# likojack/bnv_fusion

Hardware: AMD Instinct MI355X
Metric: depth frames/sec fused+decoded, 640x480 @ 256^3 grid (higher is better)
Workload: dtype f32 operands split into f16 hi+lo, 3 products on v_mfma_f32_16x16x32_f16, f32 accumulate

## Files before the change

### bnv_fusion_amd/csrc/encode.hip

```cpp
#include <stddef.h>

#include <atomic>
#include <utility>
#include <vector>

#include "frontend.hpp"

namespace bnv {

int g_num_cus = 0;
int g_last_hip_error = 0;
std::atomic<int> g_reserve_cus{0};
std::atomic<int> g_finalize_blocks{0};
std::atomic<int> g_tcnn_shared_table{1};
std::atomic<int> g_tcnn_block_encoder{1};
std::atomic<int> g_mlp_mode{1};

bool g_prof_on = false;
static std::vector<std::pair<hipEvent_t, hipEvent_t>> g_prof_events[PROF_KINDS];
static size_t g_prof_used[PROF_KINDS] = {0, 0, 0, 0};

void prof_mark(int kind, bool begin, hipStream_t stream) {
  auto& ring = g_prof_events[kind];
  if (begin) {
// ... 754 lines not shown
    lo[q] = (uint32_t)__builtin_fmaf(hf, -kFixedScale, r);
  }
#define BNV_SCAN_STEP(ctrl)                                                      \
  "v_add_co_u32_dpp %0, vcc, %0, %0 " ctrl "\n"                                  \
  "v_addc_co_u32_dpp %1, vcc, %1, %1, vcc " ctrl "\n"                            \
  "v_add_co_u32_dpp %2, vcc, %2, %2 " ctrl "\n"                                  \
  "v_addc_co_u32_dpp %3, vcc, %3, %3, vcc " ctrl "\n"                            \
  "v_add_co_u32_dpp %4, vcc, %4, %4 " ctrl "\n"                                  \
  "v_addc_co_u32_dpp %5, vcc, %5, %5, vcc " ctrl "\n"                            \
  "v_add_co_u32_dpp %6, vcc, %6, %6 " ctrl "\n"                                  \
  "v_addc_co_u32_dpp %7, vcc, %7, %7, vcc " ctrl "\n"
  asm volatile("s_nop 1\n"
               BNV_SCAN_STEP("row_shr:1 row_mask:0xf bank_mask:0xf bound_ctrl:1")
               BNV_SCAN_STEP("row_shr:2 row_mask:0xf bank_mask:0xf bound_ctrl:1")
               BNV_SCAN_STEP("row_shr:4 row_mask:0xf bank_mask:0xf bound_ctrl:1")
               BNV_SCAN_STEP("row_shr:8 row_mask:0xf bank_mask:0xf bound_ctrl:1")
               BNV_SCAN_STEP("row_bcast:15 row_mask:0xa bank_mask:0xf")
               : "+v"(lo[0]), "+v"(hi[0]), "+v"(lo[1]), "+v"(hi[1]), "+v"(lo[2]), "+v"(hi[2]), "+v"(lo[3]), "+v"(hi[3])
               :
               : "vcc");
#undef BNV_SCAN_STEP
  const int prev = __builtin_amdgcn_update_dpp(0, slot, 0x138 , 0xf, 0xf, false);
  const unsigned long long heads64 = __ballot(j == 0 || prev != slot);
  const uint32_t heads = h ? (uint32_t)(heads64 >> 32) : (uint32_t)heads64;
  const int s = 31 - __clz((int)(heads & (0xffffffffu >> (31 - j))));
  is_end = j == 31 || ((heads >> (j + 1)) & 1u);
  len = j - s + 1;
  const int src = (h * 32 + (s > 0 ? s - 1 : 0)) * 4;
#pragma unroll
  for (int q = 0; q < 4; ++q) {
    const uint32_t plo = (uint32_t)__builtin_amdgcn_ds_bpermute(src, (int)lo[q]);
    const uint32_t phi = (uint32_t)__builtin_amdgcn_ds_bpermute(src, (int)hi[q]);
    v[q] = ((unsigned long long)hi[q] << 32) | lo[q];
    if (s > 0) v[q] -= ((unsigned long long)phi << 32) | plo;
  }
}

__device__ __forceinline__ void scatter_tile(const f32x16& o, int slot, int j, int h, int32_t* __restrict__ counts,
                                             long long* __restrict__ acc) {
  unsigned long long v[4];
  bool is_end;
  int len;
  tile_run_sums(o, slot, j, h, v, is_end, len);
#ifdef BNV_PROBE_NO_SCATTER
  if ((blockIdx.x & 63) != 0) return;
#endif
  if (slot >= 0 && is_end) {
    unsigned long long* dst = (unsigned long long*)acc + ((uint32_t)slot * 8u + 4u * (uint32_t)h);
#pragma unroll
    for (int q = 0; q < 4; ++q) atomicAdd(dst + q, v[q]);
    if (h == 0) atomicAdd(&counts[slot], len);
  }
}

__global__ __launch_bounds__(512, 2) void k_pointnet_scatter(
    const float* __restrict__ pts, int n_points, bnv_grid_t g, const float* __restrict__ wpack,
    const uint32_t* __restrict__ bitmap, const uint32_t* __restrict__ word_prefix,
    int32_t* __restrict__ counts, long long* __restrict__ acc, const int32_t* __restrict__ pair_list,
    const int32_t* __restrict__ n_pairs) {
  extern __shared__ __attribute__((aligned(16))) float lds[];
  stage_to_lds<512>(wpack, lds, PN_TOTAL * 4);
  __syncthreads();

  const int lane = threadIdx.x & 63;
  const int wave = __builtin_amdgcn_readfirstlane(threadIdx.x >> 6);
  const int j = lane & 31, h = lane >> 5;
  const PairTiles T = pair_tiles(n_points, pair_list, n_pairs);
  const int n_tiles = T.n_tiles;
  const int nyz = g.n_xyz[1] * g.n_xyz[2];

  for (int t = blockIdx.x * 8 + wave; t < n_tiles; t += gridDim.x * 8) {
    int i = 0, k = 0;
    const bool have = tile_pair(T, t, j, &i, &k);
    float in0 = 0.f, in1 = 0.f, in2 = 0.f;
    int slot = -1;
    bool valid = false;
    if (have) {
      const float* p = pts + (size_t)i * 6;
      const float x = p[0], y = p[1], z = p[2];
      valid = in_bounds(x, y, z, g);
      if (valid) {
        const float xn = voxel_coord(x, g.bound_min[0], g.voxel_size);
        const float yn = voxel_coord(y, g.bound_min[1], g.voxel_size);
        const float zn = voxel_coord(z, g.bound_min[2], g.voxel_size);
        const int gx = (k & 1) ? (int)ceilf(xn) : (int)floorf(xn);
        const int gy = (k & 2) ? (int)ceilf(yn) : (int)floorf(yn);
        const int gz = (k & 4) ? (int)ceilf(zn) : (int)floorf(zn);
        if (voxel_owner(gx, gy, gz, g) == g.shard_rank) {
          const uint32_t id = (uint32_t)(gx * nyz + gy * g.n_xyz[2] + gz);
          const uint32_t word = bitmap[id >> 5];
          slot = (int)(word_prefix[id >> 5] + __popc(word & ((1u << (id & 31)) - 1u)));
        }
        const float rx = relative_coord(xn, gx, g.voxel_size);
        const float ry = relative_coord(yn, gy, g.voxel_size);
        const float rz = relative_coord(zn, gz, g.voxel_size);
        in0 = h ? ry : rx;
        in1 = h ? p[3] : rz;
        in2 = h ? p[5] : p[4];
      }
    }
    if (__ballot(slot >= 0) == 0ULL) continue;

    f32x16 ha[4], hb[4];
#pragma unroll
    for (int mb = 0; mb < 4; ++mb) ha[mb] = bias_init(lds + PN_B1, mb, h);
    {
      const float bin[3] = {in0, in1, in2};
#pragma unroll
      for (int s = 0; s < 3; ++s) {
#pragma unroll
        for (int mb = 0; mb < 4; ++mb)
          ha[mb] = __builtin_amdgcn_mfma_f32_32x32x2f32(lds[PN_W1 + (s * 4 + mb) * 64 + lane], bin[s],
                                                        ha[mb], 0, 0, 0);
      }
    }
#pragma unroll
    for (int mb = 0; mb < 4; ++mb) ha[mb] = relu16(ha[mb]);
    layer128(lds + PN_W2, lds + PN_B2, ha, hb, lane, h);
#pragma unroll
    for (int mb = 0; mb < 4; ++mb) hb[mb] = relu16(hb[mb]);
    layer128(lds + PN_W3, lds + PN_B3, hb, ha, lane, h);
#pragma unroll
    for (int mb = 0; mb < 4; ++mb) ha[mb] = relu16(ha[mb]);
    f32x16 o;
#pragma unroll
    for (int r = 0; r < 16; ++r) o[r] = 0.f;
    {
      const f32x4 b4 = *(const f32x4*)&lds[PN_B4 + 4 * h];
#pragma unroll
      for (int r = 0; r < 4; ++r) o[r] = b4[r];
    }
#pragma unroll
    for (int nb = 0; nb < 4; ++nb) {
#pragma unroll
      for (int rq = 0; rq < 4; ++rq) {
        f32x4 a = {0.f, 0.f, 0.f, 0.f};
        if (j < 8) a = *(const f32x4*)&lds[PN_W4 + ((((nb * 4 + rq) * 2 + h) * 8) + j) * 4];
#pragma unroll
        for (int i = 0; i < 4; ++i)
          o = __builtin_amdgcn_mfma_f32_32x32x2f32(a[i], ha[nb][4 * rq + i], o, 0, 0, 0);
      }
    }
    scatter_tile(o, slot, j, h, counts, acc);
  }
}


typedef _Float16 half8 __attribute__((ext_vector_type(8)));

typedef __attribute__((address_space(3))) const half8 lds_half8_t;
typedef __attribute__((address_space(3))) const f32x4 lds_f32x4_t;
constexpr int kLdsWin = 61440;

#ifdef BNV_PHASE_PROF
__device__ unsigned long long g_enc_phase[8 * 16];
#define BNV_EPH(i)                                                                          \
  do {                                                                                      \
    if ((threadIdx.x & 63) == 0) {                                                          \
      unsigned long long* _p = (unsigned long long*)((char*)lds + PX_LDS_BYTES) + (threadIdx.x >> 6) * 16; \
      const unsigned long long _t = clock64();                                              \
      _p[i] += _t - _p[15];                                                                 \
      _p[15] = _t;                                                                          \
    }                                                                                       \
  } while (0)
constexpr int kEncProfLds = 8 * 16 * 8;
#else
#define BNV_EPH(i)
constexpr int kEncProfLds = 0;
#endif

struct EncLdsX {
  uint32_t w[3];
  uint32_t b;
};
__device__ __forceinline__ half8 ldsx_wfrag(const EncLdsX& L, int byte_off) {
  const int b = byte_off / kLdsWin;
  return *(lds_half8_t*)((b == 0 ? L.w[0] : (b == 1 ? L.w[1] : L.w[2])) + (uint32_t)(byte_off - b * kLdsWin));
}
__device__ __forceinline__ f32x4 ldsx_bias(const EncLdsX& L, int layer, int rb) {
  return *(lds_f32x4_t*)(L.b + (uint32_t)((layer * 128 + rb * 16) * 4));
}

template <int NPROD>
__device__ __forceinline__ void layer128_x(const EncLdsX& L, int w_off, int layer, const half8 (&inh)[4][2],
                                           const half8 (&inl)[4][2], f32x4 (&out)[8][2]) {
#pragma unroll
  for (int rb = 0; rb < 8; ++rb) out[rb][0] = out[rb][1] = ldsx_bias(L, layer, rb);
  half8 ah[2], al[2];
#define BNV_LOAD_WX(q)                                                        \
  {                                                                           \
    const int wb = (w_off + (q) * 2 * 64 * 8) * 2;                            \
    ah[(q) & 1] = ldsx_wfrag(L, wb);                                          \
    if (NPROD == 3) al[(q) & 1] = ldsx_wfrag(L, wb + 1024);                   \
  }
  BNV_LOAD_WX(0);
#pragma unroll
  for (int q = 0; q < 32; ++q) {
    if (q + 1 < 32) BNV_LOAD_WX(q + 1);
    __builtin_amdgcn_sched_barrier(0);
    const int s = q >> 3, rb = q & 7;
    if constexpr (NPROD == 3) {
      out[rb][0] = __builtin_amdgcn_mfma_f32_16x16x32_f16(al[q & 1], inh[s][0], out[rb][0], 0, 0, 0);
      out[rb][1] = __builtin_amdgcn_mfma_f32_16x16x32_f16(al[q & 1], inh[s][1], out[rb][1], 0, 0, 0);
      out[rb][0] = __builtin_amdgcn_mfma_f32_16x16x32_f16(ah[q & 1], inl[s][0], out[rb][0], 0, 0, 0);
      out[rb][1] = __builtin_amdgcn_mfma_f32_16x16x32_f16(ah[q & 1], inl[s][1], out[rb][1], 0, 0, 0);
    }
    out[rb][0] = __builtin_amdgcn_mfma_f32_16x16x32_f16(ah[q & 1], inh[s][0], out[rb][0], 0, 0, 0);
    out[rb][1] = __builtin_amdgcn_mfma_f32_16x16x32_f16(ah[q & 1], inh[s][1], out[rb][1], 0, 0, 0);
    __builtin_amdgcn_sched_barrier(0);
  }
#undef BNV_LOAD_WX
}

template <int NPROD>
__device__ __forceinline__ void split_x(const f32x4 (&acc)[8][2], half8 (&oh)[4][2], half8 (&ol)[4][2]) {
#pragma unroll
  for (int s = 0; s < 4; ++s)
#pragma unroll
    for (int cb = 0; cb < 2; ++cb) {
      float x[8];
#pragma unroll
      for (int e = 0; e < 8; ++e) x[e] = relu_bits(acc[2 * s + (e >> 2)][cb][e & 3]);
      if (NPROD == 3) {
        split8_f16(x, oh[s][cb], ol[s][cb]);
      } else {
#pragma unroll
        for (int e = 0; e < 8; ++e) oh[s][cb][e] = (_Float16)x[e];
      }
    }
}

__device__ __forceinline__ void scatter_tile_x(const f32x4& o, int slot, int n, int g, int32_t* __restrict__ counts,
                                               long long* __restrict__ acc) {
  uint32_t lo[4], hi[4];
#pragma unroll
  for (int q = 0; q < 4; ++q) {
    const float r = __builtin_rintf(o[q] * kFixedScale);
    const float hf = __builtin_floorf(r * (1.0f / kFixedScale));
    hi[q] = (uint32_t)(int)hf;
    lo[q] = (uint32_t)__builtin_fmaf(hf, -kFixedScale, r);
  }
#define BNV_SCAN_STEP(ctrl)                                                      \
  "v_add_co_u32_dpp %0, vcc, %0, %0 " ctrl "\n"                                  \
  "v_addc_co_u32_dpp %1, vcc, %1, %1, vcc " ctrl "\n"                            \
  "v_add_co_u32_dpp %2, vcc, %2, %2 " ctrl "\n"                                  \
  "v_addc_co_u32_dpp %3, vcc, %3, %3, vcc " ctrl "\n"                            \
  "v_add_co_u32_dpp %4, vcc, %4, %4 " ctrl "\n"                                  \
  "v_addc_co_u32_dpp %5, vcc, %5, %5, vcc " ctrl "\n"                            \
  "v_add_co_u32_dpp %6, vcc, %6, %6 " ctrl "\n"                                  \
  "v_addc_co_u32_dpp %7, vcc, %7, %7, vcc " ctrl "\n"
  asm volatile("s_nop 1\n"
               BNV_SCAN_STEP("row_shr:1 row_mask:0xf bank_mask:0xf bound_ctrl:1")
               BNV_SCAN_STEP("row_shr:2 row_mask:0xf bank_mask:0xf bound_ctrl:1")
               BNV_SCAN_STEP("row_shr:4 row_mask:0xf bank_mask:0xf bound_ctrl:1")
               BNV_SCAN_STEP("row_shr:8 row_mask:0xf bank_mask:0xf bound_ctrl:1")
               : "+v"(lo[0]), "+v"(hi[0]), "+v"(lo[1]), "+v"(hi[1]), "+v"(lo[2]), "+v"(hi[2]), "+v"(lo[3]), "+v"(hi[3])
               :
               : "vcc");
#undef BNV_SCAN_STEP
  {
    const int tsrc = ((g & 1) * 16 + 15) * 4;
#pragma unroll
    for (int q = 0; q < 4; ++q) {
      const uint32_t tl = (uint32_t)__builtin_amdgcn_ds_bpermute(tsrc, (int)lo[q]);
      const uint32_t th = (uint32_t)__builtin_amdgcn_ds_bpermute(tsrc, (int)hi[q]);
      if (g >= 2) {
        const unsigned long long v = (((unsigned long long)hi[q] << 32) | lo[q]) + (((unsigned long long)th << 32) | tl);
        lo[q] = (uint32_t)v;
        hi[q] = (uint32_t)(v >> 32);
      }
    }
  }
  const int p = (g >> 1) * 16 + n;
  const int slot15 = __builtin_amdgcn_readlane(slot, 15);
  const int prev_row = __builtin_amdgcn_update_dpp(0, slot, 0x111 , 0xf, 0xf, false);
  const int prev = n == 0 ? slot15 : prev_row;
  const unsigned long long heads64 = __ballot(p == 0 || prev != slot);
  const uint32_t heads = ((uint32_t)heads64 & 0xffffu) | (((uint32_t)(heads64 >> 32) & 0xffffu) << 16);
  const int s = 31 - __clz((int)(heads & (0xffffffffu >> (31 - p))));
  const bool is_end = p == 31 || ((heads >> (p + 1)) & 1u);
  const int sp = s > 0 ? s - 1 : 0;
  const int src = (((sp >> 4) * 2 + (g & 1)) * 16 + (sp & 15)) * 4;
  uint32_t plo[4], phi[4];
#pragma unroll
  for (int q = 0; q < 4; ++q) {
    plo[q] = (uint32_t)__builtin_amdgcn_ds_bpermute(src, (int)lo[q]);
    phi[q] = (uint32_t)__builtin_amdgcn_ds_bpermute(src, (int)hi[q]);
  }
#ifdef BNV_PROBE_NO_SCATTER
  if ((blockIdx.x & 63) != 0) return;
#endif
  if (slot >= 0 && is_end) {
    unsigned long long* dst = (unsigned long long*)acc + ((uint32_t)slot * 8u + 4u * (uint32_t)(g & 1));
#pragma unroll
    for (int q = 0; q < 4; ++q) {
      unsigned long long v = ((unsigned long long)hi[q] << 32) | lo[q];
      if (s > 0) v -= ((unsigned long long)phi[q] << 32) | plo[q];
      atomicAdd(dst + q, v);
    }
    if ((g & 1) == 0) atomicAdd(&counts[slot], p - s + 1);
  }
}

template <int NPROD>
__global__ __launch_bounds__(512, 2) __attribute__((amdgpu_num_vgpr(120))) void k_pointnet_scatter_x(
    const float* __restrict__ pts, int n_points, bnv_grid_t g, const float* __restrict__ wpack,
    const uint32_t* __restrict__ bitmap, const uint32_t* __restrict__ word_prefix,
    int32_t* __restrict__ counts, long long* __restrict__ acc, int32_t* __restrict__ error,
    const int32_t* __restrict__ pair_list, const int32_t* __restrict__ n_pairs) {
  extern __shared__ __attribute__((aligned(16))) float lds[];
  const float n_cert = wpack[PN_CERT];
  float* lb = lds + PX_TOTAL / 2;
  for (int i = threadIdx.x; i < 128 * 3 + 8; i += 512) lb[i] = wpack[PN_B1 + i];
  stage_to_lds<512>(wpack + PX_OFF, lds, PX_TOTAL * 2);
  int* tile_ctr = (int*)((char*)lds + PX_TOTAL * 2 + (128 * 3 + 8) * 4);
  if (threadIdx.x == 0) *tile_ctr = 0;
  __syncthreads();

  const int lane = threadIdx.x & 63;
  const int n = lane & 15, gk = lane >> 4;
  const int pair = (gk >> 1) * 16 + n;
  const PairTiles T = pair_tiles(n_points, pair_list, n_pairs);
  const int n_tiles = T.n_tiles;
  const int nyz = g.n_xyz[1] * g.n_xyz[2];
  EncLdsX L;
  {
    const uint32_t lds0 = (uint32_t)(uintptr_t)(__attribute__((address_space(3))) float*)lds;
    L.w[0] = lds0 + lane * 16;
    L.w[1] = L.w[0] + kLdsWin;
    L.w[2] = L.w[0] + 2 * kLdsWin;
    L.b = lds0 + PX_TOTAL * 2 + gk * 16;
    asm volatile("" : "+v"(L.w[0]), "+v"(L.w[1]), "+v"(L.w[2]), "+v"(L.b));
  }

  const int tstep = gridDim.x * 8;
  auto grab = [&]() -> int {
    int c = 0;
    if (lane == 0) c = atomicAdd(tile_ctr, 1);
    c = __builtin_amdgcn_readfirstlane(c);
    return blockIdx.x * 8 + (c & 7) + (c >> 3) * tstep;
  };
  float raw[6];
  int raw_k = 0;
  bool raw_ok = false;
  float nin[6];
  uint32_t n_id = 0, n_word = 0, n_pref = 0;
  bool n_own = false;
  auto stage1 = [&](int t) {
    raw_ok = false;
    if (t < n_tiles) {
      int i = 0;
      if (tile_pair(T, t, pair, &i, &raw_k)) {
        const float* p = pts + (size_t)i * 6;
#pragma unroll
        for (int c = 0; c < 6; ++c) raw[c] = p[c];
        raw_ok = true;
      }
    }
  };
  auto stage2 = [&](int t) {
    n_own = false;
#pragma unroll
    for (int c = 0; c < 6; ++c) nin[c] = 0.f;
    if (raw_ok && in_bounds(raw[0], raw[1], raw[2], g)) {
      const int k = raw_k;
      const float xn = voxel_coord(raw[0], g.bound_min[0], g.voxel_size);
      const float yn = voxel_coord(raw[1], g.bound_min[1], g.voxel_size);
      const float zn = voxel_coord(raw[2], g.bound_min[2], g.voxel_size);
      const int gx = (k & 1) ? (int)ceilf(xn) : (int)floorf(xn);
      const int gy = (k & 2) ? (int)ceilf(yn) : (int)floorf(yn);
      const int gz = (k & 4) ? (int)ceilf(zn) : (int)floorf(zn);
      if (voxel_owner(gx, gy, gz, g) == g.shard_rank) {
        n_own = true;
        n_id = (uint32_t)(gx * nyz + gy * g.n_xyz[2] + gz);
        n_word = bitmap[n_id >> 5];
        n_pref = word_prefix[n_id >> 5];
      }
      if ((gk & 1) == 0) {
        nin[0] = relative_coord(xn, gx, g.voxel_size);
        nin[1] = relative_coord(yn, gy, g.voxel_size);
        nin[2] = relative_coord(zn, gz, g.voxel_size);
        nin[3] = raw[3];
        nin[4] = raw[4];
        nin[5] = raw[5];
      }
      if (!(fmaxf(fmaxf(fabsf(raw[3]), fabsf(raw[4])), fabsf(raw[5])) <= n_cert)) *error = 3;
    }
  };
  int t = grab();
  stage1(t);
  stage2(t);
  int t_next = grab(), t_next2 = 0;
  stage1(t_next);
#ifdef BNV_PHASE_PROF
  if ((threadIdx.x & 63) < 16)
    ((unsigned long long*)((char*)lds + PX_LDS_BYTES))[(threadIdx.x >> 6) * 16 + (threadIdx.x & 63)] = 0;
  if ((threadIdx.x & 63) == 0) ((unsigned long long*)((char*)lds + PX_LDS_BYTES))[(threadIdx.x >> 6) * 16 + 15] = clock64();
#endif

  for (; t < n_tiles; t = t_next, t_next = t_next2) {
    float in[6];
#pragma unroll
    for (int c = 0; c < 6; ++c) in[c] = nin[c];
    const int slot = n_own ? (int)(n_pref + __popc(n_word & ((1u << (n_id & 31)) - 1u))) : -1;
    stage2(t_next);
    t_next2 = grab();
    stage1(t_next2);
    __builtin_amdgcn_sched_barrier(0);
    BNV_EPH(0);
    if (__ballot(slot >= 0) == 0ULL) continue;

    f32x4 ha[8][2], hb[8][2];
    {
      half8 bh[2], bl[2];
#pragma unroll
      for (int cb = 0; cb < 2; ++cb) {
        float x[8];
#pragma unroll
        for (int e = 0; e < 8; ++e) x[e] = 0.f;
#pragma unroll
        for (int e = 0; e < 6; ++e) {
          const float other = __shfl(in[e], (lane + 32) & 63, 64);
          x[e] = gk == 0 ? (cb == 0 ? in[e] : other) : 0.f;
        }
        if (NPROD == 3) {
          split8_f16(x, bh[cb], bl[cb]);
        } else {
#pragma unroll
          for (int e = 0; e < 8; ++e) bh[cb][e] = (_Float16)x[e];
        }
      }
#pragma unroll
      for (int rb = 0; rb < 8; ++rb) {
        const half8 ahi = ldsx_wfrag(L, (PX_W1 + rb * 2 * 64 * 8) * 2), alo = ldsx_wfrag(L, (PX_W1 + rb * 2 * 64 * 8) * 2 + 1024);
        const f32x4 b = ldsx_bias(L, 0, rb);
#pragma unroll
        for (int cb = 0; cb < 2; ++cb) {
          f32x4 c = b;
          if constexpr (NPROD == 3) {
            c = __builtin_amdgcn_mfma_f32_16x16x32_f16(alo, bh[cb], c, 0, 0, 0);
            c = __builtin_amdgcn_mfma_f32_16x16x32_f16(ahi, bl[cb], c, 0, 0, 0);
          }
          ha[rb][cb] = __builtin_amdgcn_mfma_f32_16x16x32_f16(ahi, bh[cb], c, 0, 0, 0);
        }
      }
    }
    BNV_EPH(1);
    half8 sh[4][2], sl[4][2];
    split_x<NPROD>(ha, sh, sl);
    BNV_EPH(2);
    layer128_x<NPROD>(L, PX_W2, 1, sh, sl, hb);
    BNV_EPH(3);
    split_x<NPROD>(hb, sh, sl);
    BNV_EPH(4);
    layer128_x<NPROD>(L, PX_W3, 2, sh, sl, ha);
    BNV_EPH(5);
    split_x<NPROD>(ha, sh, sl);
    BNV_EPH(6);
    f32x4 o[2];
    o[0] = o[1] = *(lds_f32x4_t*)(L.b + 384 * 4);
    {
      half8 w4h[4], w4l[4];
      __builtin_amdgcn_sched_barrier(0);
#pragma unroll
      for (int s = 0; s < 4; ++s) {
        w4h[s] = ldsx_wfrag(L, (PX_W4 + s * 2 * 64 * 8) * 2);
        if (NPROD == 3) w4l[s] = ldsx_wfrag(L, (PX_W4 + s * 2 * 64 * 8) * 2 + 1024);
      }
#pragma unroll
      for (int s = 0; s < 4; ++s) {
#pragma unroll
        for (int cb = 0; cb < 2; ++cb) {
          if constexpr (NPROD == 3) {
            o[cb] = __builtin_amdgcn_mfma_f32_16x16x32_f16(w4l[s], sh[s][cb], o[cb], 0, 0, 0);
            o[cb] = __builtin_amdgcn_mfma_f32_16x16x32_f16(w4h[s], sl[s][cb], o[cb], 0, 0, 0);
          }
          o[cb] = __builtin_amdgcn_mfma_f32_16x16x32_f16(w4h[s], sh[s][cb], o[cb], 0, 0, 0);
        }
      }
    }
    f32x4 mine;
#pragma unroll
    for (int i = 0; i < 4; ++i) {
      const float other = __shfl(o[1][i], (lane + 32) & 63, 64);
      mine[i] = gk < 2 ? o[0][i] : other;
    }
    BNV_EPH(7);
    scatter_tile_x(mine, slot, n, gk, counts, acc);
    BNV_EPH(8);
  }
#ifdef BNV_PHASE_PROF
  if ((threadIdx.x & 63) < 15)
    atomicAdd(&g_enc_phase[(threadIdx.x >> 6) * 16 + (threadIdx.x & 63)],
              ((unsigned long long*)((char*)lds + PX_LDS_BYTES))[(threadIdx.x >> 6) * 16 + (threadIdx.x & 63)]);
#endif
}

constexpr int PT_W1 = 0;
constexpr int PT_W2 = PT_W1 + 2 * 64 * 8;
constexpr int PT_W3 = PT_W2 + 2 * 4 * 64 * 8;
constexpr int PT_W4 = PT_W3 + 2 * 4 * 64 * 8;
constexpr int PT_TOTAL = PT_W4 + 4 * 64 * 8;

__device__ __forceinline__ half8 to_half8_relu(const f32x16& v, int base) {
  half8 r;
#pragma unroll
  for (int e = 0; e < 8; ++e) {
    r[e] = (_Float16)relu_bits(v[base + e]);
  }
  return r;
}

__device__ __forceinline__ f32x16 zero16() {
  f32x16 v;
#pragma unroll
  for (int r = 0; r < 16; ++r) v[r] = 0.f;
  return v;
}

__global__ __launch_bounds__(256) void k_pointnet_scatter_t(
    const float* __restrict__ pts, int n_points, bnv_grid_t g, const float* __restrict__ wpack,
    const uint32_t* __restrict__ bitmap, const uint32_t* __restrict__ word_prefix,
    int32_t* __restrict__ counts, long long* __restrict__ acc, const int32_t* __restrict__ pair_list,
    const int32_t* __restrict__ n_pairs) {
  __shared__ __attribute__((aligned(16))) _Float16 wh[PT_TOTAL];
  stage_to_lds<256>(wpack, wh, PT_TOTAL * 2);
  __syncthreads();
  const int lane = threadIdx.x & 63;
  const int wave = __builtin_amdgcn_readfirstlane(threadIdx.x >> 6);
  const int j = lane & 31, h = lane >> 5;
  const PairTiles T = pair_tiles(n_points, pair_list, n_pairs);
  const int n_tiles = T.n_tiles;
  const int nyz = g.n_xyz[1] * g.n_xyz[2];
  for (int t = blockIdx.x * 4 + wave; t < n_tiles; t += gridDim.x * 4) {
    int i = 0, k = 0;
    const bool have = tile_pair(T, t, j, &i, &k);
    half8 b;
#pragma unroll
    for (int e = 0; e < 8; ++e) b[e] = (_Float16)1.0f;
    int slot = -1;
    bool valid = false;
    if (have) {
      const float* p = pts + (size_t)i * 6;
      const float x = p[0], y = p[1], z = p[2];
      if (in_bounds(x, y, z, g)) {
        valid = true;
        const float xn = voxel_coord(x, g.bound_min[0], g.voxel_size);
        const float yn = voxel_coord(y, g.bound_min[1], g.voxel_size);
        const float zn = voxel_coord(z, g.bound_min[2], g.voxel_size);
        const int gx = (k & 1) ? (int)ceilf(xn) : (int)floorf(xn);
        const int gy = (k & 2) ? (int)ceilf(yn) : (int)floorf(yn);
        const int gz = (k & 4) ? (int)ceilf(zn) : (int)floorf(zn);
        if (voxel_owner(gx, gy, gz, g) == g.shard_rank) {
          const uint32_t id = (uint32_t)(gx * nyz + gy * g.n_xyz[2] + gz);
          const uint32_t word = bitmap[id >> 5];
          slot = (int)(word_prefix[id >> 5] + __popc(word & ((1u << (id & 31)) - 1u)));
        }
        if (h == 0) {
          b[0] = (_Float16)relative_coord(xn, gx, g.voxel_size);
          b[1] = (_Float16)relative_coord(yn, gy, g.voxel_size);
          b[2] = (_Float16)relative_coord(zn, gz, g.voxel_size);
          b[3] = (_Float16)p[3];
        } else {
          b[0] = (_Float16)p[4];
          b[1] = (_Float16)p[5];
        }
      }
    }
    if (__ballot(slot >= 0) == 0ULL) continue;
    (void)valid;
    f32x16 ha[2], hb[2];
#pragma unroll
    for (int mb = 0; mb < 2; ++mb)
      ha[mb] = __builtin_amdgcn_mfma_f32_32x32x16_f16(*(const half8*)&wh[PT_W1 + (mb * 64 + lane) * 8], b, zero16(),
                                                      0, 0, 0);
    half8 s[4];
    auto layer64 = [&](int woff, const f32x16 (&in)[2], f32x16 (&out)[2]) {
#pragma unroll
      for (int nb = 0; nb < 2; ++nb) {
        s[nb * 2] = to_half8_relu(in[nb], 0);
        s[nb * 2 + 1] = to_half8_relu(in[nb], 8);
      }
#pragma unroll
      for (int mb = 0; mb < 2; ++mb) {
        out[mb] = zero16();
#pragma unroll
        for (int gk = 0; gk < 4; ++gk)
          out[mb] = __builtin_amdgcn_mfma_f32_32x32x16_f16(*(const half8*)&wh[woff + ((mb * 4 + gk) * 64 + lane) * 8],
                                                          s[gk], out[mb], 0, 0, 0);
      }
    };
    layer64(PT_W2, ha, hb);
    layer64(PT_W3, hb, ha);
#pragma unroll
    for (int nb = 0; nb < 2; ++nb) {
      s[nb * 2] = to_half8_relu(ha[nb], 0);
      s[nb * 2 + 1] = to_half8_relu(ha[nb], 8);
    }
    f32x16 o = zero16();
#pragma unroll
    for (int gk = 0; gk < 4; ++gk)
      o = __builtin_amdgcn_mfma_f32_32x32x16_f16(*(const half8*)&wh[PT_W4 + (gk * 64 + lane) * 8], s[gk], o, 0, 0, 0);
#pragma unroll
    for (int q = 0; q < 4; ++q) o[q] = (float)(_Float16)o[q];
    scatter_tile(o, slot, j, h, counts, acc);
  }
}

constexpr int kAccProbes = 6;
constexpr int kTbWaves = 8;
constexpr int kAccCap = 64 * kTbWaves;
struct WgAcc {
  int key[kAccCap];
  int cnt[kAccCap];
  unsigned long long sum[kAccCap][8];
};

template <bool SHARED>
__global__ __launch_bounds__(64 * kTbWaves) void k_pointnet_scatter_tb(
    const float* __restrict__ pts, int n_points, int frame_w, bnv_grid_t g, const float* __restrict__ wpack,
    const uint32_t* __restrict__ bitmap, const uint32_t* __restrict__ word_prefix, int32_t* __restrict__ counts,
    long long* __restrict__ acc) {
  __shared__ __attribute__((aligned(16))) _Float16 wh[PT_TOTAL];
  __shared__ WgAcc T;
  const int lane = threadIdx.x & 63;
  const int wave = __builtin_amdgcn_readfirstlane(threadIdx.x >> 6);
  constexpr int kSpan = SHARED ? kAccCap : 64;
  constexpr int kHashShift = SHARED ? 32 - 9 : 32 - 6;
  static_assert(kAccCap == 512, "hash width");
  const int t_base = SHARED ? 0 : wave * 64;
  T.key[threadIdx.x] = -1;
  T.cnt[threadIdx.x] = 0;
#pragma unroll
  for (int f = 0; f < 8; ++f) T.sum[threadIdx.x][f] = 0ull;
  stage_to_lds<64 * kTbWaves>(wpack, wh, PT_TOTAL * 2);
  __syncthreads();
  const int j = lane & 31, h = lane >> 5;
  const int nyz = g.n_xyz[1] * g.n_xyz[2];
  const bool sharded = g.shard_world > 1;
  const bool image = frame_w > 0 && n_points % frame_w == 0;
  const int frame_h = image ? n_points / frame_w : 1;
  const int bw = image ? (frame_w + 7) >> 3 : 0, bh = image ? (frame_h + 3) >> 2 : 0;
  const int n_blocks = image ? bw * bh : (n_points + 31) >> 5;
  const int uw = (bw + 1) >> 1;
  const int n_units = (SHARED && image) ? uw * ((bh + 3) >> 2) : (n_blocks + kTbWaves - 1) / kTbWaves;
  auto flush_entry = [&](int e) {
// ... 378 lines not shown

int bnv_encode_workspace_reset(void* ws, size_t ws_bytes, bnv_stream_t stream) {
  if (!ws) return BNV_ERR_INVALID_ARGUMENT;
  BNV_HIP_CHECK(hipMemsetAsync(ws, 0, ws_bytes, (hipStream_t)stream));
  return BNV_OK;
}

static bool tcnn_blocks(const bnv_grid_t& g);

static int encode_rank(const EncodeWs& ws, const bnv_grid_t& g, const float* pts, int n_points, hipStream_t stream) {
  const int nb_chunks = (int)((ws.n_chunks + kRankTile - 1) / kRankTile);
  hipLaunchKernelGGL(k_rank, dim3(nb_chunks), dim3(kScanThreads), 0, stream, ws.bytemap, ws.chunk_flag, ws.n_chunks,
                     ws.tile_state, next_epoch(), ws.bitmap, ws.word_prefix, ws.ids, ws.max_unique, ws.ctl, g,
                     ws.defer_list);
  BNV_LAUNCH_CHECK();
  if (g.shard_world > 1 && g.shard_state) {
    hipLaunchKernelGGL(k_shard_assign, dim3(1), dim3(256), 0, stream, g, (const EncCtl*)ws.ctl);
    BNV_LAUNCH_CHECK();
    const int nb = (n_points + 255) / 256;
    const int cap = 64;
    hipLaunchKernelGGL(k_shard_own, dim3(nb < cap ? (nb > 0 ? nb : 1) : cap), dim3(256), 0, stream, pts, n_points, g,
                       tcnn_blocks(g) ? (int32_t*)nullptr : ws.pair_list, &ws.ctl->n_pairs, ws.orphan_list, ws.ids,
                       ws.defer_list, ws.ctl);
    BNV_LAUNCH_CHECK();
  }
  return BNV_OK;
}

static bool tcnn_blocks(const bnv_grid_t& g) {
  return mlp_mode_of(g.mlp_mode) == 2 && g_tcnn_block_encoder.load(std::memory_order_relaxed);
}

static bool grid_ok(const bnv_grid_t& g) {
  return (int64_t)g.n_xyz[0] * g.n_xyz[1] * g.n_xyz[2] < (1LL << 31) && g.n_xyz[0] > 0 && g.n_xyz[1] > 0 &&
         g.n_xyz[2] > 0 && g.shard_world >= 1 && g.shard_world <= 64 && g.shard_rank >= 0 &&
         g.shard_rank < g.shard_world && mlp_mode_field_ok(g.mlp_mode);
}

size_t bnv_encode_shard_counts_offset(void) { return offsetof(EncCtl, shard_boundary); }

size_t bnv_shard_state_bytes(const int32_t n_xyz[3], int32_t block_log2) {
  if (!n_xyz || block_log2 < 0 || block_log2 > 8) return 0;
  return shard_state_layout(n_xyz, block_log2, nullptr, nullptr);
}
int bnv_shard_state_configure(void* shard_state, int32_t rule, int32_t axis, bnv_stream_t stream) {
  if (!shard_state || (rule != BNV_SHARD_RULE_GREEDY && rule != BNV_SHARD_RULE_REGION) || axis < 0 || axis > 2)
    return BNV_ERR_INVALID_ARGUMENT;
  const int32_t words[2] = {rule, axis};
  BNV_HIP_CHECK(hipMemcpyAsync((char*)shard_state + offsetof(ShardHdr, rule), words, sizeof(words), hipMemcpyHostToDevice,
                               (hipStream_t)stream));
  BNV_HIP_CHECK(hipStreamSynchronize((hipStream_t)stream));
  return BNV_OK;
}
size_t bnv_shard_state_loads_offset(void) { return offsetof(ShardHdr, load); }
size_t bnv_shard_state_table_offset(void) { return kShardHdrBytes; }

int bnv_encode_begin(const float* input_pts, int64_t n_points, const bnv_grid_t* grid_host, void* ws_ptr,
                     size_t ws_bytes, int64_t ws_max_points, bnv_stream_t stream_) {
  if (g_num_cus <= 0) return BNV_ERR_NOT_INITIALISED;
  if (!input_pts || !grid_host || !ws_ptr || n_points < 0 || n_points > (1 << 27) || ws_max_points < n_points)
    return BNV_ERR_INVALID_ARGUMENT;
  const bnv_grid_t g = *grid_host;
  if (!grid_ok(g)) return BNV_ERR_INVALID_ARGUMENT;
  hipStream_t stream = (hipStream_t)stream_;
  EncodeWs ws;
  if (encode_ws_layout(ws_max_points, g.n_xyz, (char*)ws_ptr, &ws) > ws_bytes) return BNV_ERR_WORKSPACE_TOO_SMALL;
  if (n_points == 0) return BNV_OK;
  const int n = (int)n_points;
  hipLaunchKernelGGL(k_mark, dim3((n + 255) / 256), dim3(256), 0, stream, input_pts, n, g, ws.bytemap, ws.chunk_flag,
                     ws.valid_blocks,
                     (g.shard_world > 1 && !tcnn_blocks(g)) ? ws.pair_list : (int32_t*)nullptr, &ws.ctl->n_pairs,
                     g.shard_state ? ws.orphan_list : (int32_t*)nullptr, &ws.ctl->n_orphans);
  BNV_LAUNCH_CHECK();
  return encode_rank(ws, g, input_pts, n, stream);
}

int bnv_encode_begin_depth(const void* depth, int depth_dtype, int H, int W, const double* intr_host,
                           const double* T_wc_host, double max_depth, const bnv_grid_t* grid_host, void* ws_ptr,
                           size_t ws_bytes, int64_t ws_max_points, float* out_pts, bnv_stream_t stream_) {
  if (g_num_cus <= 0) return BNV_ERR_NOT_INITIALISED;
  if (!depth || !intr_host || !T_wc_host || !grid_host || !ws_ptr || !out_pts || H <= 0 || W <= 0 || depth_dtype < 0 ||
      depth_dtype > 2 || (int64_t)H * W > (1 << 27) || ws_max_points < (int64_t)H * W)
    return BNV_ERR_INVALID_ARGUMENT;
  const bnv_grid_t g = *grid_host;
  if (!grid_ok(g)) return BNV_ERR_INVALID_ARGUMENT;
  hipStream_t stream = (hipStream_t)stream_;
  EncodeWs ws;
  if (encode_ws_layout(ws_max_points, g.n_xyz, (char*)ws_ptr, &ws) > ws_bytes) return BNV_ERR_WORKSPACE_TOO_SMALL;
  FrontArgs a;
  front_args_fill(a, depth, depth_dtype, H, W, intr_host, T_wc_host, max_depth);
  const int64_t n = (int64_t)H * W;
  hipLaunchKernelGGL(k_front_mark, dim3((unsigned)((n + 255) / 256)), dim3(256), 0, stream, a, out_pts, g, ws.bytemap,
                     ws.chunk_flag, ws.valid_blocks,
                     (g.shard_world > 1 && !tcnn_blocks(g)) ? ws.pair_list : (int32_t*)nullptr, &ws.ctl->n_pairs,
                     g.shard_state ? ws.orphan_list : (int32_t*)nullptr, &ws.ctl->n_orphans);
  BNV_LAUNCH_CHECK();
  return encode_rank(ws, g, out_pts, (int)n, stream);
}

int bnv_encode_finish(const float* input_pts, int64_t n_points, const bnv_grid_t* grid_host,
                      const float* pointnet_pack, void* ws_ptr, size_t ws_bytes, int64_t ws_max_points,
                      float* out_feats, int64_t* out_pcounts, int64_t* out_flat_ids, int64_t* out_grid_ids,
                      int64_t out_capacity, int emit_all, bnv_encode_counters_t* counters, bnv_stream_t stream) {
  return bnv_encode_finish_image(input_pts, n_points, 0, grid_host, pointnet_pack, ws_ptr, ws_bytes, ws_max_points,
                                 out_feats, out_pcounts, out_flat_ids, out_grid_ids, out_capacity, emit_all, counters,
                                 stream);
}

int bnv_encode_finish_image(const float* input_pts, int64_t n_points, int image_width, const bnv_grid_t* grid_host,
                            const float* pointnet_pack, void* ws_ptr, size_t ws_bytes, int64_t ws_max_points,
                            float* out_feats, int64_t* out_pcounts, int64_t* out_flat_ids, int64_t* out_grid_ids,
                            int64_t out_capacity, int emit_all, bnv_encode_counters_t* counters, bnv_stream_t stream_) {
  return bnv_encode_finish_image_wg(input_pts, n_points, image_width, grid_host, pointnet_pack, ws_ptr, ws_bytes,
                                    ws_max_points, out_feats, out_pcounts, out_flat_ids, out_grid_ids, out_capacity,
                                    emit_all, counters, 0, stream_);
}

int bnv_encode_finish_image_wg(const float* input_pts, int64_t n_points, int image_width, const bnv_grid_t* grid_host,
                               const float* pointnet_pack, void* ws_ptr, size_t ws_bytes, int64_t ws_max_points,
                               float* out_feats, int64_t* out_pcounts, int64_t* out_flat_ids, int64_t* out_grid_ids,
                               int64_t out_capacity, int emit_all, bnv_encode_counters_t* counters,
                               int max_workgroups, bnv_stream_t stream_) {
  return bnv_encode_finish_image_parts(input_pts, n_points, image_width, grid_host, pointnet_pack, ws_ptr, ws_bytes,
                                       ws_max_points, out_feats, out_pcounts, out_flat_ids, out_grid_ids, out_capacity,
                                       emit_all, counters, max_workgroups, 3, stream_);
}

int bnv_encode_finish_image_parts(const float* input_pts, int64_t n_points, int image_width,
                                  const bnv_grid_t* grid_host, const float* pointnet_pack, void* ws_ptr,
                                  size_t ws_bytes, int64_t ws_max_points, float* out_feats, int64_t* out_pcounts,
                                  int64_t* out_flat_ids, int64_t* out_grid_ids, int64_t out_capacity, int emit_all,
                                  bnv_encode_counters_t* counters, int max_workgroups, int parts,
                                  bnv_stream_t stream_) {
  if (g_num_cus <= 0) return BNV_ERR_NOT_INITIALISED;
  if (image_width < 0 || max_workgroups < 0 || parts < 1 || parts > 3) return BNV_ERR_INVALID_ARGUMENT;
  if (!input_pts || !grid_host || !pointnet_pack || !ws_ptr || !counters || n_points < 0 ||
      n_points > (1 << 27) || ws_max_points < n_points)
    return BNV_ERR_INVALID_ARGUMENT;
  const bnv_grid_t g = *grid_host;
  if (!grid_ok(g)) return BNV_ERR_INVALID_ARGUMENT;
  hipStream_t stream = (hipStream_t)stream_;
  EncodeWs ws;
  if (encode_ws_layout(ws_max_points, g.n_xyz, (char*)ws_ptr, &ws) > ws_bytes) return BNV_ERR_WORKSPACE_TOO_SMALL;
  if (n_points == 0) {
    if (parts & 2) BNV_HIP_CHECK(hipMemsetAsync(counters, 0, sizeof(bnv_encode_counters_t), stream));
    return BNV_OK;
  }
  const int n = (int)n_points;
  const int n_tiles = ((n + 31) / 32) * 8;
  const int reserve = g_reserve_cus.load(std::memory_order_relaxed);
  int grid_pn = g_num_cus - reserve > 0 ? g_num_cus - reserve : 1;
  if (max_workgroups > 0 && grid_pn > max_workgroups) grid_pn = max_workgroups;
  if (grid_pn > (n_tiles + 7) / 8) grid_pn = (n_tiles + 7) / 8;
  const int mlp = mlp_mode_of(g.mlp_mode);
  const int32_t* plist = (g.shard_world > 1 && !tcnn_blocks(g)) ? ws.pair_list : (const int32_t*)nullptr;
  if (parts & 1) {
    ProfScope prof(PROF_POINTNET, stream);
    if (tcnn_blocks(g)) {
      const int n_blocks = (n + 31) / 32 + 64;
      const int n_units = (n_blocks + kTbWaves - 1) / kTbWaves + 64;
      const int cus_tb = max_workgroups > 0 && max_workgroups < g_num_cus ? max_workgroups : g_num_cus;
      const int grid_tb = cus_tb * 2 < n_units ? cus_tb * 2 : n_units;
      auto kern = g_tcnn_shared_table.load(std::memory_order_relaxed) ? k_pointnet_scatter_tb<true> : k_pointnet_scatter_tb<false>;
      hipLaunchKernelGGL(kern, dim3(grid_tb), dim3(64 * kTbWaves), 0, stream, input_pts, n, image_width, g,
                         pointnet_pack, ws.bitmap, ws.word_prefix, ws.counts, ws.acc);
    } else if (mlp == 2)
      hipLaunchKernelGGL(k_pointnet_scatter_t, dim3(g_num_cus * 4 < (n_tiles + 3) / 4 ? g_num_cus * 4 : (n_tiles + 3) / 4),
                         dim3(256), 0, stream, input_pts, n, g, pointnet_pack, ws.bitmap, ws.word_prefix, ws.counts,
                         ws.acc, plist, &ws.ctl->n_pairs);
    else if (mlp == 1) {
      hipLaunchKernelGGL((k_pointnet_scatter_x<3>), dim3(grid_pn), dim3(512), PX_LDS_BYTES + kEncProfLds, stream,
                         input_pts, n, g, pointnet_pack, ws.bitmap, ws.word_prefix, ws.counts, ws.acc, &ws.ctl->error,
                         plist, &ws.ctl->n_pairs);
    } else if (mlp == 3) {
      hipLaunchKernelGGL((k_pointnet_scatter_x<1>), dim3(grid_pn), dim3(512), PX_LDS_BYTES + kEncProfLds, stream,
                         input_pts, n, g, pointnet_pack, ws.bitmap, ws.word_prefix, ws.counts, ws.acc, &ws.ctl->error,
                         plist, &ws.ctl->n_pairs);
    } else
      hipLaunchKernelGGL(k_pointnet_scatter, dim3(grid_pn), dim3(512), PN_TOTAL * 4, stream, input_pts, n, g,
                         pointnet_pack, ws.bitmap, ws.word_prefix, ws.counts, ws.acc, plist, &ws.ctl->n_pairs);
  }
  BNV_LAUNCH_CHECK();
  if (!(parts & 2)) return BNV_OK;
  const int nb_max = (int)((ws.max_unique + kFinTile - 1) / kFinTile);
  const int nb_res = 2 * g_num_cus;
  const int nb_opt = g_finalize_blocks.load(std::memory_order_relaxed);
  const int nb_cap = nb_opt > 0 && nb_opt < nb_res ? nb_opt : nb_res;
  const int nb_u = nb_max < nb_cap ? nb_max : nb_cap;
  hipLaunchKernelGGL(k_finalize, dim3(nb_u), dim3(kFinTile), 0, stream, g, emit_all, ws.bitmap, ws.ids,
                     ws.counts, ws.acc, ws.tile_state, next_epoch(), ws.ctl, ws.valid_blocks, (n + 255) / 256, out_feats,
                     out_pcounts, out_flat_ids, out_grid_ids, out_capacity, counters);
  BNV_LAUNCH_CHECK();
  return BNV_OK;
}

int bnv_encode_pointcloud(const float* input_pts, int64_t n_points, const bnv_grid_t* grid_host,
                          const float* pointnet_pack, void* ws_ptr, size_t ws_bytes, int64_t ws_max_points,
                          float* out_feats,
                          int64_t* out_pcounts, int64_t* out_flat_ids, int64_t* out_grid_ids,
                          int64_t out_capacity, int emit_all, bnv_encode_counters_t* counters,
                          bnv_stream_t stream) {
  if (!pointnet_pack || !counters) return BNV_ERR_INVALID_ARGUMENT;
  const int rc = bnv_encode_begin(input_pts, n_points, grid_host, ws_ptr, ws_bytes, ws_max_points, stream);
  if (rc != BNV_OK) return rc;
  return bnv_encode_finish(input_pts, n_points, grid_host, pointnet_pack, ws_ptr, ws_bytes, ws_max_points, out_feats,
                           out_pcounts, out_flat_ids, out_grid_ids, out_capacity, emit_all, counters, stream);
}

int bnv_voxelize_pairs(const float* input_pts, int64_t n_points, const bnv_grid_t* grid_host,
                       int32_t* grid_ids, int64_t* flat_ids, float* rel_xyz, uint8_t* bound_mask,
                       bnv_stream_t stream) {
  if (!input_pts || !grid_host || n_points < 0 || n_points > (1 << 27)) return BNV_ERR_INVALID_ARGUMENT;
  if (n_points == 0) return BNV_OK;
  hipLaunchKernelGGL(k_voxelize_pairs, dim3((unsigned)((n_points + 255) / 256)), dim3(256), 0,
                     (hipStream_t)stream, input_pts, (int)n_points, *grid_host, grid_ids, flat_ids, rel_xyz,
                     bound_mask);
  BNV_LAUNCH_CHECK();
  return BNV_OK;
}

}
```

Baseline: 573.1.

## Interleave hi/lo split and next-layer weight loads with MFMA chains in PointNet MLP

Restructures the MLP layers so each 16-row block's accumulators are finished one at a time and then split into f16 hi/lo while the next block's MFMAs run. The last layer's products are folded into the third layer. Weight fragments are double-buffered, and sched_group_barrier hints interleave VALU, LDS reads and MFMA. This removes the separate split passes and the full 8x2 f32 accumulator arrays, which lowers register pressure and lets the explicit 120-VGPR cap be dropped. The wave count per block also becomes a compile-time knob. The risks are scheduling-hint fragility and changed occupancy now that the VGPR cap is gone.

```diff
diff --git a/bnv_fusion_amd/csrc/encode.hip b/bnv_fusion_amd/csrc/encode.hip
--- a/bnv_fusion_amd/csrc/encode.hip
+++ b/bnv_fusion_amd/csrc/encode.hip
@@ -930,6 +930,11 @@
 typedef __attribute__((address_space(3))) const f32x4 lds_f32x4_t;
 constexpr int kLdsWin = 61440;
 
+#ifndef BNV_PX_WAVES
+#define BNV_PX_WAVES 8
+#endif
+constexpr int kPxWaves = BNV_PX_WAVES;
+
 #ifdef BNV_PHASE_PROF
 __device__ unsigned long long g_enc_phase[8 * 16];
 #define BNV_EPH(i)                                                                          \
@@ -941,7 +946,7 @@
       _p[15] = _t;                                                                          \
     }                                                                                       \
   } while (0)
-constexpr int kEncProfLds = 8 * 16 * 8;
+constexpr int kEncProfLds = kPxWaves * 16 * 8;
 #else
 #define BNV_EPH(i)
 constexpr int kEncProfLds = 0;
@@ -960,52 +965,100 @@
 }
 
 template <int NPROD>
-__device__ __forceinline__ void layer128_x(const EncLdsX& L, int w_off, int layer, const half8 (&inh)[4][2],
-                                           const half8 (&inl)[4][2], f32x4 (&out)[8][2]) {
-#pragma unroll
-  for (int rb = 0; rb < 8; ++rb) out[rb][0] = out[rb][1] = ldsx_bias(L, layer, rb);
+__device__ __forceinline__ void split_rb_x(const f32x4 (&acc)[2], int rb, half8 (&oh)[4][2], half8 (&ol)[4][2]) {
+  typedef unsigned u32x4_t __attribute__((ext_vector_type(4)));
+#pragma unroll
+  for (int cb = 0; cb < 2; ++cb) {
+    float x[4];
+#pragma unroll
+    for (int i = 0; i < 4; ++i) x[i] = relu_bits(acc[cb][i]);
+    if constexpr (NPROD == 3) {
+      u32x4_t h = __builtin_bit_cast(u32x4_t, oh[rb >> 1][cb]), l = __builtin_bit_cast(u32x4_t, ol[rb >> 1][cb]);
+      unsigned h0, l0, h1, l1;
+      split_pair_f16(x[0], x[1], h0, l0);
+      split_pair_f16(x[2], x[3], h1, l1);
+      h[2 * (rb & 1)] = h0;
+      h[2 * (rb & 1) + 1] = h1;
+      l[2 * (rb & 1)] = l0;
+      l[2 * (rb & 1) + 1] = l1;
+      oh[rb >> 1][cb] = __builtin_bit_cast(half8, h);
+      ol[rb >> 1][cb] = __builtin_bit_cast(half8, l);
+    } else {
+#pragma unroll
+      for (int i = 0; i < 4; ++i) oh[rb >> 1][cb][4 * (rb & 1) + i] = (_Float16)x[i];
+    }
+  }
+}
+
+template <int NPROD, int VALU>
+__device__ __forceinline__ void sched_step_x(bool loads) {
+#pragma unroll
+  for (int m = 0; m < 2 * NPROD; ++m) {
+    __builtin_amdgcn_sched_group_barrier(0x008, 1, 0);
+    if (loads && m < NPROD) __builtin_amdgcn_sched_group_barrier(0x100, 1, 0);
+    if (m + 1 < 2 * NPROD) __builtin_amdgcn_sched_group_barrier(0x002, VALU, 0);
+  }
+}
+
+template <int NPROD, bool L4>
+__device__ __forceinline__ void layer128_x(const EncLdsX& L, int w_off, int layer, half8 (&inh)[4][2],
+                                           half8 (&inl)[4][2], half8 (&oh)[4][2], half8 (&ol)[4][2],
+                                           f32x4 (&pend)[2], f32x4 (&o4)[2], half8 (&w4)[2]) {
   half8 ah[2], al[2];
-#define BNV_LOAD_WX(q)                                                        \
+#define BNV_LOAD_WX(s, rb)                                                    \
   {                                                                           \
-    const int wb = (w_off + (q) * 2 * 64 * 8) * 2;                            \
-    ah[(q) & 1] = ldsx_wfrag(L, wb);                                          \
-    if (NPROD == 3) al[(q) & 1] = ldsx_wfrag(L, wb + 1024);                   \
-  }
-  BNV_LOAD_WX(0);
-#pragma unroll
-  for (int q = 0; q < 32; ++q) {
-    if (q + 1 < 32) BNV_LOAD_WX(q + 1);
+    const int wb = (w_off + ((s) * 8 + (rb)) * 2 * 64 * 8) * 2;               \
+    ah[(s) & 1] = ldsx_wfrag(L, wb);                                          \
+    if (NPROD == 3) al[(s) & 1] = ldsx_wfrag(L, wb + 1024);                   \
+  }
+  BNV_LOAD_WX(0, 0);
+#pragma unroll
+  for (int rb = 0; rb < 8; ++rb) {
+    f32x4 acc[2];
+    const f32x4 b = ldsx_bias(L, layer, rb);
+#pragma unroll
+    for (int s = 0; s < 4; ++s) {
+      if (s + 1 < 4) BNV_LOAD_WX(s + 1, rb) else if (rb + 1 < 8) BNV_LOAD_WX(0, rb + 1);
+#pragma unroll
+      for (int cb = 0; cb < 2; ++cb) {
+        f32x4 c = s == 0 ? b : acc[cb];
+        if constexpr (NPROD == 3) {
+          c = __builtin_amdgcn_mfma_f32_16x16x32_f16(al[s & 1], inh[s][cb], c, 0, 0, 0);
+          c = __builtin_amdgcn_mfma_f32_16x16x32_f16(ah[s & 1], inl[s][cb], c, 0, 0, 0);
+        }
+        acc[cb] = __builtin_amdgcn_mfma_f32_16x16x32_f16(ah[s & 1], inh[s][cb], c, 0, 0, 0);
+      }
+      if (s < 3) {
+        if (s == 0) split_rb_x<NPROD>(pend, rb == 0 ? 7 : rb - 1, rb == 0 ? inh : oh, rb == 0 ? inl : ol);
+        sched_step_x<NPROD, NPROD == 3 ? 2 : 3>(s + 1 < 4 || rb + 1 < 8);
+      } else {
+        sched_step_x<NPROD, 0>(rb + 1 < 8);
+      }
+    }
+    if constexpr (L4) {
+      __builtin_amdgcn_sched_barrier(0);
+      if (rb >= 3 && (rb & 1)) {
+        const int s4 = (rb - 3) >> 1;
+#pragma unroll
+        for (int cb = 0; cb < 2; ++cb) {
+          if constexpr (NPROD == 3) {
+            o4[cb] = __builtin_amdgcn_mfma_f32_16x16x32_f16(w4[1], oh[s4][cb], o4[cb], 0, 0, 0);
+            o4[cb] = __builtin_amdgcn_mfma_f32_16x16x32_f16(w4[0], ol[s4][cb], o4[cb], 0, 0, 0);
+          }
+          o4[cb] = __builtin_amdgcn_mfma_f32_16x16x32_f16(w4[0], oh[s4][cb], o4[cb], 0, 0, 0);
+        }
+      }
+      if ((rb >= 2 && !(rb & 1)) || rb == 7) {
+        const int s4 = (rb - 1) >> 1;
+        w4[0] = ldsx_wfrag(L, (PX_W4 + s4 * 2 * 64 * 8) * 2);
+        if (NPROD == 3) w4[1] = ldsx_wfrag(L, (PX_W4 + s4 * 2 * 64 * 8) * 2 + 1024);
+      }
+    }
+    pend[0] = acc[0];
+    pend[1] = acc[1];
     __builtin_amdgcn_sched_barrier(0);
-    const int s = q >> 3, rb = q & 7;
-    if constexpr (NPROD == 3) {
-      out[rb][0] = __builtin_amdgcn_mfma_f32_16x16x32_f16(al[q & 1], inh[s][0], out[rb][0], 0, 0, 0);
-      out[rb][1] = __builtin_amdgcn_mfma_f32_16x16x32_f16(al[q & 1], inh[s][1], out[rb][1], 0, 0, 0);
-      out[rb][0] = __builtin_amdgcn_mfma_f32_16x16x32_f16(ah[q & 1], inl[s][0], out[rb][0], 0, 0, 0);
-      out[rb][1] = __builtin_amdgcn_mfma_f32_16x16x32_f16(ah[q & 1], inl[s][1], out[rb][1], 0, 0, 0);
-    }
-    out[rb][0] = __builtin_amdgcn_mfma_f32_16x16x32_f16(ah[q & 1], inh[s][0], out[rb][0], 0, 0, 0);
-    out[rb][1] = __builtin_amdgcn_mfma_f32_16x16x32_f16(ah[q & 1], inh[s][1], out[rb][1], 0, 0, 0);
-    __builtin_amdgcn_sched_barrier(0);
   }
 #undef BNV_LOAD_WX
-}
-
-template <int NPROD>
-__device__ __forceinline__ void split_x(const f32x4 (&acc)[8][2], half8 (&oh)[4][2], half8 (&ol)[4][2]) {
-#pragma unroll
-  for (int s = 0; s < 4; ++s)
-#pragma unroll
-    for (int cb = 0; cb < 2; ++cb) {
-      float x[8];
-#pragma unroll
-      for (int e = 0; e < 8; ++e) x[e] = relu_bits(acc[2 * s + (e >> 2)][cb][e & 3]);
-      if (NPROD == 3) {
-        split8_f16(x, oh[s][cb], ol[s][cb]);
-      } else {
-#pragma unroll
-        for (int e = 0; e < 8; ++e) oh[s][cb][e] = (_Float16)x[e];
-      }
-    }
 }
 
 __device__ __forceinline__ void scatter_tile_x(const f32x4& o, int slot, int n, int g, int32_t* __restrict__ counts,
@@ -1081,7 +1134,7 @@
 }
 
 template <int NPROD>
-__global__ __launch_bounds__(512, 2) __attribute__((amdgpu_num_vgpr(120))) void k_pointnet_scatter_x(
+__global__ __launch_bounds__(64 * kPxWaves, kPxWaves / 4) void k_pointnet_scatter_x(
     const float* __restrict__ pts, int n_points, bnv_grid_t g, const float* __restrict__ wpack,
     const uint32_t* __restrict__ bitmap, const uint32_t* __restrict__ word_prefix,
     int32_t* __restrict__ counts, long long* __restrict__ acc, int32_t* __restrict__ error,
@@ -1089,8 +1142,8 @@
   extern __shared__ __attribute__((aligned(16))) float lds[];
   const float n_cert = wpack[PN_CERT];
   float* lb = lds + PX_TOTAL / 2;
-  for (int i = threadIdx.x; i < 128 * 3 + 8; i += 512) lb[i] = wpack[PN_B1 + i];
-  stage_to_lds<512>(wpack + PX_OFF, lds, PX_TOTAL * 2);
+  for (int i = threadIdx.x; i < 128 * 3 + 8; i += 64 * kPxWaves) lb[i] = wpack[PN_B1 + i];
+  stage_to_lds<64 * kPxWaves>(wpack + PX_OFF, lds, PX_TOTAL * 2);
   int* tile_ctr = (int*)((char*)lds + PX_TOTAL * 2 + (128 * 3 + 8) * 4);
   if (threadIdx.x == 0) *tile_ctr = 0;
   __syncthreads();
@@ -1111,12 +1164,12 @@
     asm volatile("" : "+v"(L.w[0]), "+v"(L.w[1]), "+v"(L.w[2]), "+v"(L.b));
   }
 
-  const int tstep = gridDim.x * 8;
+  const int tstep = gridDim.x * kPxWaves;
   auto grab = [&]() -> int {
     int c = 0;
     if (lane == 0) c = atomicAdd(tile_ctr, 1);
     c = __builtin_amdgcn_readfirstlane(c);
-    return blockIdx.x * 8 + (c & 7) + (c >> 3) * tstep;
+    return blockIdx.x * kPxWaves + c % kPxWaves + c / kPxWaves * tstep;
   };
   float raw[6];
   int raw_k = 0;
@@ -1188,9 +1241,10 @@
     BNV_EPH(0);
     if (__ballot(slot >= 0) == 0ULL) continue;
 
-    f32x4 ha[8][2], hb[8][2];
+    half8 ah[4][2], al[4][2], bh[4][2], bl[4][2];
+    f32x4 pend[2];
     {
-      half8 bh[2], bl[2];
+      half8 xh[2], xl[2];
 #pragma unroll
       for (int cb = 0; cb < 2; ++cb) {
         float x[8];
@@ -1202,74 +1256,79 @@
           x[e] = gk == 0 ? (cb == 0 ? in[e] : other) : 0.f;
         }
         if (NPROD == 3) {
-          split8_f16(x, bh[cb], bl[cb]);
+          split8_f16(x, xh[cb], xl[cb]);
         } else {
 #pragma unroll
-          for (int e = 0; e < 8; ++e) bh[cb][e] = (_Float16)x[e];
+          for (int e = 0; e < 8; ++e) xh[cb][e] = (_Float16)x[e];
         }
       }
+      __builtin_amdgcn_sched_barrier(0);
+      asm volatile("s_nop 1");
+      __builtin_amdgcn_sched_barrier(0);
+      half8 whi = ldsx_wfrag(L, PX_W1 * 2), wlo = ldsx_wfrag(L, PX_W1 * 2 + 1024);
 #pragma unroll
       for (int rb = 0; rb < 8; ++rb) {
-        const half8 ahi = ldsx_wfrag(L, (PX_W1 + rb * 2 * 64 * 8) * 2), alo = ldsx_wfrag(L, (PX_W1 + rb * 2 * 64 * 8) * 2 + 1024);
+        const half8 hi = whi, lo = wlo;
+        if (rb + 1 < 8) {
+          whi = ldsx_wfrag(L, (PX_W1 + (rb + 1) * 2 * 64 * 8) * 2);
+          wlo = ldsx_wfrag(L, (PX_W1 + (rb + 1) * 2 * 64 * 8) * 2 + 1024);
+        }
         const f32x4 b = ldsx_bias(L, 0, rb);
+        f32x4 acc[2];
 #pragma unroll
         for (int cb = 0; cb < 2; ++cb) {
           f32x4 c = b;
           if constexpr (NPROD == 3) {
-            c = __builtin_amdgcn_mfma_f32_16x16x32_f16(alo, bh[cb], c, 0, 0, 0);
-            c = __builtin_amdgcn_mfma_f32_16x16x32_f16(ahi, bl[cb], c, 0, 0, 0);
+            c = __builtin_amdgcn_mfma_f32_16x16x32_f16(lo, xh[cb], c, 0, 0, 0);
+            c = __builtin_amdgcn_mfma_f32_16x16x32_f16(hi, xl[cb], c, 0, 0, 0);
           }
-          ha[rb][cb] = __builtin_amdgcn_mfma_f32_16x16x32_f16(ahi, bh[cb], c, 0, 0, 0);
+          acc[cb] = __builtin_amdgcn_mfma_f32_16x16x32_f16(hi, xh[cb], c, 0, 0, 0);
         }
+        if (rb > 0) split_rb_x<NPROD>(pend, rb - 1, ah, al);
+        pend[0] = acc[0];
+        pend[1] = acc[1];
+#pragma unroll
+        for (int m = 0; m < 2 * NPROD; ++m) {
+          __builtin_amdgcn_sched_group_barrier(0x008, 1, 0);
+          if (m < 2) __builtin_amdgcn_sched_group_barrier(0x100, 1, 0);
+          if (m + 1 < 2 * NPROD) __builtin_amdgcn_sched_group_barrier(0x002, NPROD == 3 ? 5 : 12, 0);
+        }
+        __builtin_amdgcn_sched_barrier(0);
       }
     }
     BNV_EPH(1);
-    half8 sh[4][2], sl[4][2];
-    split_x<NPROD>(ha, sh, sl);
+    f32x4 o[2];
+    half8 w4[2];
+    layer128_x<NPROD, false>(L, PX_W2, 1, ah, al, bh, bl, pend, o, w4);
     BNV_EPH(2);
-    layer128_x<NPROD>(L, PX_W2, 1, sh, sl, hb);
+    o[0] = o[1] = *(lds_f32x4_t*)(L.b + 384 * 4);
+    layer128_x<NPROD, true>(L, PX_W3, 2, bh, bl, ah, al, pend, o, w4);
+    split_rb_x<NPROD>(pend, 7, ah, al);
+    __builtin_amdgcn_sched_barrier(0);
+    asm volatile("s_nop 1");
+    __builtin_amdgcn_sched_barrier(0);
+#pragma unroll
+    for (int cb = 0; cb < 2; ++cb) {
+      if constexpr (NPROD == 3) {
+        o[cb] = __builtin_amdgcn_mfma_f32_16x16x32_f16(w4[1], ah[3][cb], o[cb], 0, 0, 0);
+        o[cb] = __builtin_amdgcn_mfma_f32_16x16x32_f16(w4[0], al[3][cb], o[cb], 0, 0, 0);
+      }
+      o[cb] = __builtin_amdgcn_mfma_f32_16x16x32_f16(w4[0], ah[3][cb], o[cb], 0, 0, 0);
+    }
     BNV_EPH(3);
-    split_x<NPROD>(hb, sh, sl);
-    BNV_EPH(4);
-    layer128_x<NPROD>(L, PX_W3, 2, sh, sl, ha);
-    BNV_EPH(5);
-    split_x<NPROD>(ha, sh, sl);
-    BNV_EPH(6);
-    f32x4 o[2];
-    o[0] = o[1] = *(lds_f32x4_t*)(L.b + 384 * 4);
-    {
-      half8 w4h[4], w4l[4];
-      __builtin_amdgcn_sched_barrier(0);
-#pragma unroll
-      for (int s = 0; s < 4; ++s) {
-        w4h[s] = ldsx_wfrag(L, (PX_W4 + s * 2 * 64 * 8) * 2);
-        if (NPROD == 3) w4l[s] = ldsx_wfrag(L, (PX_W4 + s * 2 * 64 * 8) * 2 + 1024);
-      }
-#pragma unroll
-      for (int s = 0; s < 4; ++s) {
-#pragma unroll
-        for (int cb = 0; cb < 2; ++cb) {
-          if constexpr (NPROD == 3) {
-            o[cb] = __builtin_amdgcn_mfma_f32_16x16x32_f16(w4l[s], sh[s][cb], o[cb], 0, 0, 0);
-            o[cb] = __builtin_amdgcn_mfma_f32_16x16x32_f16(w4h[s], sl[s][cb], o[cb], 0, 0, 0);
-          }
-          o[cb] = __builtin_amdgcn_mfma_f32_16x16x32_f16(w4h[s], sh[s][cb], o[cb], 0, 0, 0);
-        }
-      }
-    }
     f32x4 mine;
 #pragma unroll
     for (int i = 0; i < 4; ++i) {
       const float other = __shfl(o[1][i], (lane + 32) & 63, 64);
       mine[i] = gk < 2 ? o[0][i] : other;
     }
-    BNV_EPH(7);
+    BNV_EPH(4);
     scatter_tile_x(mine, slot, n, gk, counts, acc);
-    BNV_EPH(8);
+    BNV_EPH(5);
   }
 #ifdef BNV_PHASE_PROF
   if ((threadIdx.x & 63) < 15)
-    atomicAdd(&g_enc_phase[(threadIdx.x >> 6) * 16 + (threadIdx.x & 63)],
+    atomicAdd(&g_enc_phase[((threadIdx.x >> 6) & 7) * 16 + (threadIdx.x & 63)],
               ((unsigned long long*)((char*)lds + PX_LDS_BYTES))[(threadIdx.x >> 6) * 16 + (threadIdx.x & 63)]);
 #endif
 }
@@ -1954,6 +2013,7 @@
   int grid_pn = g_num_cus - reserve > 0 ? g_num_cus - reserve : 1;
   if (max_workgroups > 0 && grid_pn > max_workgroups) grid_pn = max_workgroups;
   if (grid_pn > (n_tiles + 7) / 8) grid_pn = (n_tiles + 7) / 8;
+  const int grid_px = grid_pn < (n_tiles + kPxWaves - 1) / kPxWaves ? grid_pn : (n_tiles + kPxWaves - 1) / kPxWaves;
   const int mlp = mlp_mode_of(g.mlp_mode);
   const int32_t* plist = (g.shard_world > 1 && !tcnn_blocks(g)) ? ws.pair_list : (const int32_t*)nullptr;
   if (parts & 1) {
@@ -1971,11 +2031,11 @@
                          dim3(256), 0, stream, input_pts, n, g, pointnet_pack, ws.bitmap, ws.word_prefix, ws.counts,
                          ws.acc, plist, &ws.ctl->n_pairs);
     else if (mlp == 1) {
-      hipLaunchKernelGGL((k_pointnet_scatter_x<3>), dim3(grid_pn), dim3(512), PX_LDS_BYTES + kEncProfLds, stream,
+      hipLaunchKernelGGL((k_pointnet_scatter_x<3>), dim3(grid_px), dim3(64 * kPxWaves), PX_LDS_BYTES + kEncProfLds, stream,
                          input_pts, n, g, pointnet_pack, ws.bitmap, ws.word_prefix, ws.counts, ws.acc, &ws.ctl->error,
                          plist, &ws.ctl->n_pairs);
     } else if (mlp == 3) {
-      hipLaunchKernelGGL((k_pointnet_scatter_x<1>), dim3(grid_pn), dim3(512), PX_LDS_BYTES + kEncProfLds, stream,
+      hipLaunchKernelGGL((k_pointnet_scatter_x<1>), dim3(grid_px), dim3(64 * kPxWaves), PX_LDS_BYTES + kEncProfLds, stream,
                          input_pts, n, g, pointnet_pack, ws.bitmap, ws.word_prefix, ws.counts, ws.acc, &ws.ctl->error,
                          plist, &ws.ctl->n_pairs);
     } else
```

Measured after the change: 575.5 (median of 6 runs). Within noise of the previous version (+0.4%).
